# TopJohn/corda

Hardware: AMD Instinct MI355X
Metric: signature verifications/sec (whole node, 1/2/4/8 GPU) + % integer-ALU peak (higher is better)
Workload: dtype u32

## Files before the change

### corda_amd/csrc/ed25519.hip

```cpp
#ifndef FE_QUAD
#define FE_QUAD 0
#endif
#ifndef FE_USE_ASM2
#define FE_USE_ASM2 1
#endif
#include <hip/hip_runtime.h>

#include <functional>
#include <stdint.h>
#include <stdlib.h>

#include "ed25519_half.hpp"
#include "ed25519_ops.hpp"
#include "ed25519_route.hpp"
#include "ed25519_ws.hpp"
#include "sha2_device.hpp"
#include "status.hpp"

namespace cordahip {

__global__ void __launch_bounds__(64) ed25519_btable_kernel(uint32_t* __restrict__ tab) {
  const int g = blockIdx.x * blockDim.x + threadIdx.x;
  if (g >= 2 * kBTableEntries) return;
  const int k = g % kBTableEntries;
  ge_p3 B, P;
  ge_base(B);
  if (g >= kBTableEntries)
    for (int t = 0; t < kBDigits * kBBits; t++) ge_dbl<true>(B, B);
  ge_cached bc;
  ge_to_cached(bc, B);
  ge_identity(P);
  for (int bit = kBBits - 1; bit >= 0; bit--) {
    ge_dbl<true>(P, P);
    if ((k >> bit) & 1) ge_add<true>(P, P, bc);
  }
  store_niels_entry(tab + g * kBEntryWords, P);
  if (g == 0) {
    ge_cached id;
    fe_set(id.YpX, 1);
    fe_set(id.YmX, 1);
    fe_set(id.Z, 1);
    fe_set(id.T2d, 0);
    store_cached(tab + kBIdentityWord, id);
  }
}


CDEV double mp8_top(const uint32_t a[8], int s) {
  const int w = s >> 5, b = s & 31;
  const uint64_t lo = ((uint64_t)word_sel(a, w + 1) << 32) | word_sel(a, w);
  const uint64_t hi = word_sel(a, w + 2);
  return (double)((lo >> b) | (b ? hi << (64 - b) : 0ull));
}
CDEV void mp8_lincomb(uint32_t o[8], const uint32_t x[8], int a, const uint32_t y[8], int b) {
  const uint32_t ua = (uint32_t)(a < 0 ? -a : a), ub = (uint32_t)(b < 0 ? -b : b);
  uint64_t pc = 0, qc = 0;
  uint32_t br = 0;
#pragma unroll
  for (int i = 0; i < 8; i++) {
    const uint64_t p = (uint64_t)ua * x[i] + pc;
    pc = p >> 32;
    const uint64_t q = (uint64_t)ub * y[i] + qc;
    qc = q >> 32;
    const uint64_t d = (uint64_t)(uint32_t)p - (uint32_t)q - br;
    o[i] = (uint32_t)d;
    br = (uint32_t)(d >> 63);
  }
  if (b > 0 || (b == 0 && a < 0)) mp8_neg(o);
}

CDEV void half_scalars(uint32_t c0abs[8], bool& c0neg, uint32_t c1[8], const uint32_t h[8]) {
  const uint32_t kM[8] = {0xe7ae9f68u, 0xc09318d2u, 0x17bce6b2u, 0xa6f7cef5u, 0u, 0u, 0u, 0x80000000u};
  const uint32_t kS[8] = {0x754abea0u, 0x597d89b3u, 0xf9de6484u, 0xb504f333u, 0u, 0u, 0u, 0u};
  uint32_t rp[8], rc[8], tp[8], tc[8];
#pragma unroll
  for (int i = 0; i < 8; i++) {
    rp[i] = kM[i];
    rc[i] = h[i];
    tp[i] = 0;
    tc[i] = i == 0;
  }
  for (;;) {
    const int s = max(mp8_bitlen(rp) - 52, 0);
    double uh = mp8_top(rp, s), vh = mp8_top(rc, s);
    const double th = mp8_top(kS, s) + 1.0;
    double A = 1.0, B = 0.0, C = 0.0, D = 1.0;
    int n = 0;
    for (;;) {
      const double d1 = vh + C, d2 = vh + D;
      if (!(d1 > 0.0 && d2 > 0.0)) break;
      const double n1 = uh + A;
      double q = floor(n1 / d1);
      const double r1 = fma(-q, d1, n1);
      q = r1 < 0.0 ? q - 1.0 : (r1 >= d1 ? q + 1.0 : q);
      const double r2 = fma(-q, d2, uh + B);
      if (!(r2 >= 0.0 && r2 < d2)) break;
      const double nC = fma(-q, C, A), nD = fma(-q, D, B), nv = fma(-q, vh, uh);
      const double mc = fmax(fabs(nC), fabs(nD));
      if (nv - mc < th || mc >= 0x1p30) break;
      A = C;
      B = D;
      C = nC;
      D = nD;
      uh = vh;
      vh = nv;
      n++;
    }
    if (n == 0) break;
    const int a = (int)A, b = (int)B, c = (int)C, d = (int)D;
    uint32_t x[8], y[8];
    mp8_lincomb(x, rp, a, rc, b);
// ... 172 lines not shown
  ge_to_cached(c, E);
  store_cached(joint_slot(rec, joint_index(2, 2 * s)), c);
}


#ifndef ED_PREP_WAVES
#define ED_PREP_WAVES 2
#endif
CDEV uint8_t prep_decode_phase(const uint8_t* __restrict__ keys, const uint8_t* __restrict__ sigs, uint64_t i,
                               uint32_t msg_len, const uint8_t* __restrict__ pre_status, uint32_t empty_is_error,
                               uint32_t* __restrict__ rec, uint32_t* col, uint32_t abyte[8], uint32_t Rw[8]) {
  uint8_t st = kStatusPending;
  load8(Rw, reinterpret_cast<const uint32_t*>(sigs + i * 64));
  {
    uint32_t wa[8];
    load8(wa, reinterpret_cast<const uint32_t*>(keys + i * 32));
    ge_p3 A, R;
    bool okA, okR;
    ge_frombytes_i2p_pair(A, okA, wa, R, okR, Rw);
    if (!okA) st = kStatusBadKey;
    else if (pre_status && pre_status[i] != kStatusOk) st = pre_status[i];
    else if (msg_len == 0 && empty_is_error) st = kStatusEmpty;
    fe_tobytes(abyte, A.Y);
    abyte[7] |= fe_isnegative(A.X) << 31;
    if (st == kStatusPending && !(okR && ge_strict_ok(R, Rw))) st = kStatusBadSig;
    if (st != kStatusPending) {
      ge_identity(A);
      ge_identity(R);
    }
    fe_neg(A.X, A.X);
    fe_neg(A.T, A.T);
    fe_neg(R.X, R.X);
    fe_neg(R.T, R.T);
    park_point(rec, col, 0, A);
    park_point(rec, col, 1, R);
  }
  return st;
}

CDEV void prep_table_phase(uint32_t* __restrict__ rec, uint32_t* col) {
#pragma unroll 1
  for (int pass = 0; pass < 2; pass++) {
    joint_single_pass(rec, col, pass);
    PHASE_BARRIER();
  }
#pragma unroll 1
  for (int s = -1; s <= 1; s += 2) {
    joint_sign_pass(rec, col, s);
    PHASE_BARRIER();
  }
}

CDEV uint8_t prep_keys_phase(const uint8_t* __restrict__ keys, const uint8_t* __restrict__ sigs, uint64_t i,
                             uint32_t msg_len, const uint8_t* __restrict__ pre_status, uint32_t empty_is_error,
                             uint32_t* __restrict__ rec, uint32_t* col, uint32_t abyte[8], uint32_t Rw[8]) {
  const uint8_t st = prep_decode_phase(keys, sigs, i, msg_len, pre_status, empty_is_error, rec, col, abyte, Rw);
  PHASE_BARRIER();
  prep_table_phase(rec, col);
  return st;
}

CDEV void prep_msg_phase(const uint8_t* __restrict__ sigs, const uint8_t* __restrict__ msgs, uint32_t msg_len,
                         uint64_t i, uint8_t st, const uint32_t abyte[8], const uint32_t Rw[8],
                         uint32_t* __restrict__ rec) {
  uint32_t ka[8], kr[8], e[8];
  bool c0neg = false;
  if (st == kStatusPending) {
    uint32_t S[8], hd[16], h[8], se[8], zero[8];
    load8(S, reinterpret_cast<const uint32_t*>(sigs + i * 64 + 32));
    sha512_segments(hd, Rw, abyte, true, msgs + i * (uint64_t)msg_len, msg_len);
    sc_reduce512(h, hd);
    sc_effective_S(se, S, slide_drops_carry(S));
    half_scalars(ka, c0neg, kr, h);
#pragma unroll
    for (int q = 0; q < 8; q++) zero[q] = 0;
    sc_muladd(e, kr, se, zero);
  } else {
#pragma unroll
    for (int q = 0; q < 8; q++) ka[q] = kr[q] = e[q] = 0;
  }
#if ED_SEL_STREAM
  uint32_t sel[32];
  sel_recode(sel, ka, kr, e, c0neg);
  sel[kSelWords] = 0;
  uint4* o4 = reinterpret_cast<uint4*>(rec + kWhSel);
#pragma unroll
  for (int q = 0; q < 8; q++) o4[q] = make_uint4(sel[4 * q], sel[4 * q + 1], sel[4 * q + 2], sel[4 * q + 3]);
#else
  store8(rec + kWhKa, ka);
  store8(rec + kWhKr, kr);
  store8(rec + kWhE, e);
  reinterpret_cast<uint4*>(rec + kWhFlags)[0] = make_uint4(c0neg ? 1u : 0u, 0u, 0u, 0u);
#endif
}

#if ED_PREP_LDS
#define PREP_PARK_COLUMN(col)                  \
  __shared__ uint32_t pq_lds[kPqWords][256]; \
  uint32_t* col = &pq_lds[0][threadIdx.x]
#else
#define PREP_PARK_COLUMN(col) uint32_t* col = nullptr
#endif

__global__ void __launch_bounds__(256) __attribute__((amdgpu_waves_per_eu(ED_PREP_WAVES))) ed25519_prep_half_kernel(
    const uint8_t* __restrict__ keys, const uint8_t* __restrict__ sigs, const uint8_t* __restrict__ msgs,
    uint32_t msg_len, uint64_t base, uint64_t m, const uint8_t* __restrict__ pre_status,
    uint8_t* __restrict__ status, uint32_t* __restrict__ ws, uint32_t empty_is_error) {
  const uint64_t li = (uint64_t)blockIdx.x * blockDim.x + threadIdx.x;
  if (li >= m) return;
  const uint64_t i = base + li;
  uint32_t* rec = ws + li * kWhLaneWords;
  uint32_t abyte[8], Rw[8];
  PREP_PARK_COLUMN(col);
  const uint8_t st = prep_keys_phase(keys, sigs, i, msg_len, pre_status, empty_is_error, rec, col, abyte, Rw);
  prep_msg_phase(sigs, msgs, msg_len, i, st, abyte, Rw, rec);
  status[i] = st;
}

__global__ void __launch_bounds__(256) __attribute__((amdgpu_waves_per_eu(ED_PREP_WAVES)))
ed25519_prep_half_idx_kernel(const uint8_t* __restrict__ keys, const uint8_t* __restrict__ sigs,
                             const uint8_t* __restrict__ msgs, uint32_t msg_len, uint64_t base, uint64_t m,
                             const uint8_t* __restrict__ pre_status, uint8_t* __restrict__ status,
                             uint32_t* __restrict__ ws, uint32_t empty_is_error, const uint32_t* __restrict__ scratch,
                             uint64_t lanes) {
  const uint64_t li = (uint64_t)blockIdx.x * blockDim.x + threadIdx.x;
  if (li >= route_chunk_lanes(scratch[kRouteCntGeneric], base, m)) return;
  const uint64_t i = scratch[route_off_generic(lanes) + base + li];
  uint32_t* rec = ws + li * kWhLaneWords;
  uint32_t abyte[8], Rw[8];
  PREP_PARK_COLUMN(col);
  const uint8_t st = prep_keys_phase(keys, sigs, i, msg_len, pre_status, empty_is_error, rec, col, abyte, Rw);
  prep_msg_phase(sigs, msgs, msg_len, i, st, abyte, Rw, rec);
  status[i] = st;
}

__global__ void __launch_bounds__(256) __attribute__((amdgpu_waves_per_eu(ED_PREP_WAVES))) ed25519_prep_keys_kernel(
    const uint8_t* __restrict__ keys, const uint8_t* __restrict__ sigs, uint32_t msg_len, uint64_t base, uint64_t m,
    const uint8_t* __restrict__ pre_status, uint8_t* __restrict__ status, uint32_t* __restrict__ ws,
    uint32_t empty_is_error) {
  const uint64_t li = (uint64_t)blockIdx.x * blockDim.x + threadIdx.x;
  if (li >= m) return;
  const uint64_t i = base + li;
  uint32_t* rec = ws + li * kWhLaneWords;
  uint32_t abyte[8], Rw[8];
  PREP_PARK_COLUMN(col);
  status[i] = prep_keys_phase(keys, sigs, i, msg_len, pre_status, empty_is_error, rec, col, abyte, Rw);
  store8(rec + kWhKa, abyte);
}

__global__ void __launch_bounds__(256) __attribute__((amdgpu_waves_per_eu(ED_PREP_WAVES))) ed25519_prep_msg_kernel(const uint8_t* __restrict__ sigs,
                                                               const uint8_t* __restrict__ msgs, uint32_t msg_len,
                                                               uint64_t base, uint64_t m,
                                                               const uint8_t* __restrict__ status,
                                                               uint32_t* __restrict__ ws) {
  const uint64_t li = (uint64_t)blockIdx.x * blockDim.x + threadIdx.x;
  if (li >= m) return;
  const uint64_t i = base + li;
  uint32_t* rec = ws + li * kWhLaneWords;
  uint32_t abyte[8], Rw[8];
  load8(abyte, rec + kWhKa);
  load8(Rw, reinterpret_cast<const uint32_t*>(sigs + i * 64));
  prep_msg_phase(sigs, msgs, msg_len, i, status[i], abyte, Rw, rec);
}

CDEV void fixed_base_mult(ge_p3& P, const uint32_t k[8], const uint32_t* __restrict__ btab) {
  ge_identity(P);
  for (int j = 31; j >= 0; j--) {
// ... 143 lines not shown
```

### corda_amd/csrc/ed25519_ladder.hip

```cpp
#ifndef FE_USE_ASM2
#define FE_USE_ASM2 1
#endif
#include <hip/hip_runtime.h>
#include <stdint.h>

#include "ed25519_route.hpp"
#include "ed25519_ws.hpp"
#include "status.hpp"

namespace cordahip {

__device__ __attribute__((aligned(64))) const uint32_t kIdentityCached[kWhEntryWords] = {1, 0, 0, 0, 0, 0, 0, 0, 0, 0,
                                                            1, 0, 0, 0, 0, 0, 0, 0, 0, 0,
                                                            1, 0, 0, 0, 0, 0, 0, 0, 0, 0,
                                                            0, 0, 0, 0, 0, 0, 0, 0, 0, 0};

#ifndef ED_LADDER_WAVES
#define ED_LADDER_WAVES 2
#endif
static_assert(512 / ED_LADDER_WAVES >= 168, "fe25519_asm.hpp's v160..v167 accumulators need >= 168 VGPRs per lane");

#ifndef ED_LADDER_ORDER
#define ED_LADDER_ORDER 1
#endif
#if ED_LADDER_ORDER && !ED_SEL_STREAM
#error "ED_LADDER_ORDER ranks the lanes by the selector stream's window count"
#endif
static constexpr int kOrderLo = 60, kOrderHi = 74, kOrderKeys = kOrderHi - kOrderLo + 2;
static_assert(kOrderKeys <= 64, "one lane of a wave per key");

template <bool kIdx>
CDEV void ladder_half_lane(uint64_t base, uint64_t m, const uint32_t* __restrict__ btab,
                           const uint32_t* __restrict__ ws, uint8_t* __restrict__ status,
                           unsigned long long* __restrict__ verdict, const uint32_t* __restrict__ list) {
  const uint64_t blk = (uint64_t)blockIdx.x * blockDim.x;
#if ED_LADDER_ORDER
  __shared__ uint32_t sk[kSelWords][256];
  __shared__ uint8_t order_src[256];
  __shared__ uint32_t order_cnt[4][kOrderKeys];
  __shared__ uint32_t order_done;
  uint64_t li;
  {
    const uint64_t l0 = blk + threadIdx.x;
    const uint32_t* r0 = ws + (l0 < m ? l0 : m - 1) * kWhLaneWords;
    const uint4* r4 = reinterpret_cast<const uint4*>(r0 + kWhSel);
    uint4 v[(kSelWords + 3) / 4];
#pragma unroll
    for (int q = 0; q < (kSelWords + 3) / 4; q++) v[q] = r4[q];
    static_assert(kSelMeta == 30 && (kSelWords + 3) / 4 == 8, "the count is in the last quad's third word");
    const int cnt = (int)(v[7].z >> 16);
    const int key = l0 < m ? min(max(cnt, kOrderLo), kOrderHi) - kOrderLo : kOrderKeys - 1;
    const int lane = threadIdx.x & 63, wave = threadIdx.x >> 6;
    uint32_t before = 0, mine = 0;
#pragma unroll
    for (int k = 0; k < kOrderKeys; k++) {
      const unsigned long long mk = __ballot(key == k);
      if (key == k) before = (uint32_t)__popcll(mk & ((1ull << lane) - 1));
      if (lane == k) mine = (uint32_t)__popcll(mk);
    }
    if (lane < kOrderKeys) order_cnt[wave][lane] = mine;
    if (threadIdx.x == 0) order_done = 0;
    __syncthreads();
    uint32_t rank = before;
#pragma unroll
    for (int k = 0; k < kOrderKeys; k++)
#pragma unroll
      for (int w = 0; w < 4; w++) {
        const uint32_t c = order_cnt[w][k];
        rank += (k < key || (k == key && w < wave)) ? c : 0u;
      }
    order_src[rank] = (uint8_t)threadIdx.x;
#pragma unroll
    for (int q = 0; q < (kSelWords + 3) / 4; q++) {
      const uint32_t w[4] = {v[q].x, v[q].y, v[q].z, v[q].w};
#pragma unroll
      for (int t = 0; t < 4; t++)
        if (4 * q + t < kSelWords) sk[4 * q + t][rank] = w[t];
    }
    __syncthreads();
    li = blk + order_src[threadIdx.x];
  }
#else
  const uint64_t li = blk + threadIdx.x;
#endif
  const bool active = li < m;
  const uint64_t lc = active ? li : m - 1;
  const uint32_t* rec = ws + lc * kWhLaneWords;
#if ED_IDENT_GLOBAL
  const uint32_t* ident = btab + kBIdentityWord;
#else
  const uint32_t* ident = kIdentityCached;
#endif
  const uint32_t* btab2 = btab + kBTableEntries * kBEntryWords;
  ge_p3 P;
  ge_identity(P);
#if ED_SEL_STREAM
#if !ED_LADDER_ORDER
  __shared__ uint32_t sk[kSelWords][256];
  {
    const uint4* r4 = reinterpret_cast<const uint4*>(rec + kWhSel);
#pragma unroll
    for (int q = 0; q < (kSelWords + 3) / 4; q++) {
      const uint4 v = r4[q];
      const uint32_t w[4] = {v.x, v.y, v.z, v.w};
#pragma unroll
      for (int t = 0; t < 4; t++)
        if (4 * q + t < kSelWords) sk[4 * q + t][threadIdx.x] = w[t];
    }
  }
#endif
  const uint32_t* col = &sk[0][threadIdx.x];
#if ED_LADDER_ORDER
  const int own = active ? (int)(col[kSelMeta * 256] >> 16) : 0;
#else
  const int own = (int)(col[kSelMeta * 256] >> 16);
#endif
  const int W = min(max(wave_max(own), (kBDigits - 1) * (kBBits / 2) + 1), kSelWindows);
  uint32_t selw = col[((W - 1) / kSelPerWord) * 256];
  for (int j = W - 1; j >= 0; j--) {
    const int jn = max(j - 1, 0);
    const uint32_t selw_next = col[(jn / kSelPerWord) * 256];
    const uint32_t sel = selw >> (kSelBits * (j % kSelPerWord));
    const uint32_t idx = sel & 15u;
    const bool neg = sel & kSelNeg;
    ge_cached c;
    load_cached(c, idx == kSelIdentity ? ident : rec + kWhTab + idx * kWhEntryWords);
    const bool bwin = j % (kBBits / 2) == 0 && j < kBDigits * (kBBits / 2);
    uint32_t m0 = 0, m1 = 0, sg = 0;
    const int t = j / (kBBits / 2);
    if (bwin) {
      m0 = col[(kSelMag + (t >> 1)) * 256];
      m1 = col[(kSelMag + ((t + kBDigits) >> 1)) * 256];
      sg = col[kSelMeta * 256];
    }
    if (j != W - 1) {
      ge_dbl<false>(P, P);
      ge_dbl<true>(P, P);
    }
    cached_cneg(c, neg);
    if (bwin) {
      const int sh = 16 * (t & 1);
      ge_niels nb0, nb1;
      uint32_t pad0[2], pad1[2];
      load_niels(nb0, btab, (int)((m0 >> sh) & 0xffffu), pad0);
      ge_add<true>(P, P, c);
      load_niels(nb1, btab2, (int)((m1 >> sh) & 0xffffu), pad1);
      niels_pad_use(pad0);
      niels_cneg(nb0, (sg >> t) & 1u);
      ge_madd<true>(P, P, nb0);
      niels_pad_use(pad1);
      niels_cneg(nb1, (sg >> (t + kBDigits)) & 1u);
      ge_madd<false>(P, P, nb1);
    } else {
      ge_add<false>(P, P, c);
    }
    selw = selw_next;
  }
#else
  __shared__ uint32_t sk[24][256];
  const uint32_t* ska = &sk[0][threadIdx.x];
  const uint32_t* skr = &sk[8][threadIdx.x];
  const uint32_t* ske = &sk[16][threadIdx.x];
  int bits;
  {
    uint32_t ka[8], kr[8], e[8];
    load8(ka, rec + kWhKa);
    load8(kr, rec + kWhKr);
    load8(e, rec + kWhE);
#pragma unroll
    for (int q = 0; q < 8; q++) {
      sk[q][threadIdx.x] = ka[q];
      sk[8 + q][threadIdx.x] = kr[q];
      sk[16 + q][threadIdx.x] = e[q];
    }
    bits = max(mp8_bitlen(ka), mp8_bitlen(kr));
  }
  const bool c0neg = rec[kWhFlags] & 1u;
  const int W = max(wave_max((bits + 2) / 2), (kBDigits - 1) * (kBBits / 2) + 1);
  for (int j = W - 1; j >= 0; j--) {
    const joint_sel sel = joint_select(joint_booth2(ska, 256, 8, j), joint_booth2(skr, 256, 8, j), c0neg);
    ge_cached c;
    load_cached(c, table_entry(rec, sel.idx, ident));
    if (j != W - 1) {
      ge_dbl<false>(P, P);
      ge_dbl<true>(P, P);
    }
    cached_cneg(c, sel.neg);
    const bool bwin = j % (kBBits / 2) == 0 && j < kBDigits * (kBBits / 2);
    if (bwin) {
      const int d0 = booth_digit_col<kBBits>(ske, j / (kBBits / 2));
      const int d1 = booth_digit_col<kBBits>(ske, j / (kBBits / 2) + kBDigits);
      ge_niels nb0, nb1;
      load_niels(nb0, btab, d0 < 0 ? -d0 : d0);
      ge_add<true>(P, P, c);
      load_niels(nb1, btab2, d1 < 0 ? -d1 : d1);
      niels_cneg(nb0, d0 < 0);
      ge_madd<true>(P, P, nb0);
      niels_cneg(nb1, d1 < 0);
      ge_madd<false>(P, P, nb1);
    } else {
      ge_add<false>(P, P, c);
    }
  }
#endif
  fe d;
  fe_sub(d, P.Y, P.Z);
  const bool zero = fe_iszero(P.X) && fe_iszero(d);
  const uint64_t i = kIdx ? (active ? list[base + li] : 0) : base + li;
  uint8_t st = kStatusBadSig;
  if (active) {
    st = status[i];
    if (st == kStatusPending) {
      st = zero ? kStatusOk : kStatusBadSig;
      status[i] = st;
    }
  }
  if (!kIdx) {
#if ED_LADDER_ORDER
    __shared__ uint8_t order_ok[256];
    order_ok[li - blk] = active && st == kStatusOk;
    __builtin_amdgcn_fence(__ATOMIC_RELEASE, "workgroup");
    uint32_t arrived = 0;
    if ((threadIdx.x & 63) == 0)
      arrived = __hip_atomic_fetch_add(&order_done, 1u, __ATOMIC_RELAXED, __HIP_MEMORY_SCOPE_WORKGROUP);
    arrived = (uint32_t)__shfl((int)arrived, 0);
    if (arrived == blockDim.x / 64 - 1) {
      __builtin_amdgcn_fence(__ATOMIC_ACQUIRE, "workgroup");
      const int lane = threadIdx.x & 63;
#pragma unroll
      for (int q = 0; q < 4; q++) {
        const unsigned long long ok = __ballot(order_ok[64 * q + lane] != 0);
        if (lane == q && blk + 64 * q < m && verdict) verdict[(base + blk + 64 * q) >> 6] = ok;
      }
    }
#else
    const unsigned long long ok = __ballot(active && st == kStatusOk);
    if ((threadIdx.x & 63) == 0 && active && verdict) verdict[i >> 6] = ok;
#endif
  }
}

__global__ void __launch_bounds__(256) __attribute__((amdgpu_waves_per_eu(ED_LADDER_WAVES))) ed25519_ladder_half_kernel(
    uint64_t base, uint64_t m, const uint32_t* __restrict__ btab, const uint32_t* __restrict__ ws,
    uint8_t* __restrict__ status, unsigned long long* __restrict__ verdict) {
  ladder_half_lane<false>(base, m, btab, ws, status, verdict, nullptr);
}

__global__ void __launch_bounds__(256) __attribute__((amdgpu_waves_per_eu(ED_LADDER_WAVES)))
ed25519_ladder_half_idx_kernel(uint64_t base, uint64_t m, const uint32_t* __restrict__ btab,
                               const uint32_t* __restrict__ ws, uint8_t* __restrict__ status,
                               const uint32_t* __restrict__ scratch, uint64_t lanes) {
  const uint64_t mm = route_chunk_lanes(scratch[kRouteCntGeneric], base, m);
  if ((uint64_t)blockIdx.x * blockDim.x >= mm) return;
  ladder_half_lane<true>(base, mm, btab, ws, status, nullptr, scratch + route_off_generic(lanes));
}

hipError_t launch_ed25519_ladder(uint64_t base, uint64_t m, const uint32_t* btab, const uint32_t* ws, uint8_t* status,
                                 unsigned long long* verdict, hipStream_t s) {
  const uint32_t blocks = (uint32_t)((m + 255) / 256);
  hipLaunchKernelGGL(ed25519_ladder_half_kernel, dim3(blocks), dim3(256), 0, s, base, m, btab, ws, status, verdict);
  return hipGetLastError();
}

hipError_t launch_ed25519_ladder_idx(uint64_t base, uint64_t m, const uint32_t* btab, const uint32_t* ws,
                                     uint8_t* status, const uint32_t* scratch, uint64_t lanes, hipStream_t s) {
  const uint32_t blocks = (uint32_t)((m + 255) / 256);
  hipLaunchKernelGGL(ed25519_ladder_half_idx_kernel, dim3(blocks), dim3(256), 0, s, base, m, btab, ws, status, scratch,
                     lanes);
  return hipGetLastError();
}

}
```

### corda_amd/csrc/ed25519_sel.hpp

```cpp
#pragma once
#include <stdint.h>

#include "ed25519_joint.hpp"

namespace cordahip {

static constexpr int kSelPerWord = 6, kSelBits = 5;
static constexpr int kSelWindows = 132;
static constexpr uint32_t kSelIdentity = 15;
static constexpr uint32_t kSelNeg = 16;
static constexpr int kSelBDigits = 16;
static constexpr int kSelMag = kSelWindows / kSelPerWord;
static constexpr int kSelMeta = kSelMag + kSelBDigits / 2;
static constexpr int kSelWords = kSelMeta + 1;
static constexpr int kSelAlways = 80;
static_assert(kSelWindows % kSelPerWord == 0 && kSelWindows >= 129 && kSelWords <= 32,
              "the stream lives in the record's 32 scalar words");

static constexpr uint32_t kBooth2Lut = 2u | 3u << 3 | 3u << 6 | 4u << 9 | 0u << 12 | 1u << 15 | 1u << 18 | 2u << 21;

JOINT_HD uint32_t sel_byte(uint32_t va, uint32_t vr) {
  const int ta = (int)((kBooth2Lut >> (3 * va)) & 7u), tr = (int)((kBooth2Lut >> (3 * vr)) & 7u);
  const int s = 5 * ta + tr - 12;
  const int m = s < 0 ? -s : s;
  return ((uint32_t)(m - 1) & 15u) | (s < 0 ? kSelNeg : 0u);
}
static_assert(((uint32_t)kJointIdentity & 15u) == kSelIdentity && kJointEntries <= (int)kSelIdentity &&
                  (kSelNeg | 15u) < (1u << kSelBits),
              "selector encoding");

JOINT_HD void sel_word(uint32_t out[kSelWords], int w, uint32_t a, uint32_t r, uint32_t pa, uint32_t pr) {
#pragma unroll
  for (int b = 0; b < 16; b++) {
    const int j = 16 * w + b;
    if (j >= kSelWindows) break;
    const uint32_t va = b ? (a >> (2 * b - 1)) & 7u : ((a << 1) | pa) & 7u;
    const uint32_t vr = b ? (r >> (2 * b - 1)) & 7u : ((r << 1) | pr) & 7u;
    const int sh = kSelBits * (j % kSelPerWord);
    out[j / kSelPerWord] ^= (sel_byte(va, vr) ^ (j >= kSelAlways ? kSelIdentity : 0u)) << sh;
  }
}

JOINT_HD void sel_recode(uint32_t out[kSelWords], const uint32_t c0abs[8], const uint32_t c1[8], const uint32_t e[8],
                         bool c0neg) {
  const uint32_t flip = c0neg ? ~0u : 0u;
#pragma unroll
  for (int k = 0; k < kSelMag; k++) {
    uint32_t v = 0;
#pragma unroll
    for (int t = 0; t < kSelPerWord; t++)
      if (kSelPerWord * k + t >= kSelAlways) v |= kSelIdentity << (kSelBits * t);
    out[k] = v;
  }
#pragma unroll
  for (int w = 0; w < kSelAlways / 16; w++)
    sel_word(out, w, c0abs[w] ^ flip, c1[w], w ? (c0abs[w - 1] ^ flip) >> 31 : flip >> 31, w ? c1[w - 1] >> 31 : 0u);
  const uint32_t high = (c0abs[4] | c1[4]) >> 31 | c0abs[5] | c1[5] | c0abs[6] | c1[6] | c0abs[7] | c1[7];
  if (high) {
#pragma unroll
    for (int w = kSelAlways / 16; w <= 8; w++)
      sel_word(out, w, (w < 8 ? c0abs[w] : 0u) ^ flip, w < 8 ? c1[w] : 0u, (c0abs[w - 1] ^ flip) >> 31, c1[w - 1] >> 31);
  }
  uint32_t signs = 0;
#pragma unroll
  for (int w = 0; w < kSelBDigits / 2; w++) {
    const uint32_t v0 = ((e[w] << 1) | (w ? e[w - 1] >> 31 : 0u)) & 0x1ffffu, v1 = e[w] >> 15;
    const int d0 = (int)((v0 + 1) >> 1) - (int)((v0 >> 16) << 16), d1 = (int)((v1 + 1) >> 1) - (int)((v1 >> 16) << 16);
    signs |= (d0 < 0 ? 1u : 0u) << (2 * w) | (d1 < 0 ? 1u : 0u) << (2 * w + 1);
    out[kSelMag + w] = (uint32_t)(d0 < 0 ? -d0 : d0) | (uint32_t)(d1 < 0 ? -d1 : d1) << 16;
  }
  int bits = 0;
#pragma unroll
  for (int i = 0; i < 8; i++) {
    const uint32_t m = c0abs[i] | c1[i];
    bits = m ? 32 * i + 32 - __builtin_clz(m) : bits;
  }
  out[kSelMeta] = signs | (uint32_t)((bits + 2) / 2) << 16;
}

JOINT_HD uint32_t sel_window(const uint32_t s[kSelWords], int j) {
  return (s[j / kSelPerWord] >> (kSelBits * (j % kSelPerWord))) & ((1u << kSelBits) - 1);
}
JOINT_HD int sel_count(const uint32_t s[kSelWords]) { return (int)((s[kSelMeta] >> 16) & 0xffu); }
JOINT_HD int sel_bdigit(const uint32_t s[kSelWords], int t) {
  const int mag = (int)((s[kSelMag + (t >> 1)] >> (16 * (t & 1))) & 0xffffu);
  return (s[kSelMeta] >> t) & 1u ? -mag : mag;
}

}
```

### corda_amd/csrc/ed25519_ws.hpp

```cpp
#pragma once
#include "ed25519_joint.hpp"
#include "ed25519_sel.hpp"
#include "fe25519.hpp"
#include "ge25519.hpp"
#include "sc25519.hpp"

namespace cordahip {

static constexpr int kBBits = 16;
static constexpr int kBDigits = 8;
static constexpr int kBTableEntries = (1 << (kBBits - 1)) + 1;
static constexpr int kBEntryWords = 32;
static constexpr int kBIdentityWord = 2 * kBTableEntries * kBEntryWords;
static_assert(kSelBDigits == 2 * kBDigits, "ed25519_sel.hpp recodes both halves of e");
static constexpr uint8_t kStatusPending = 0xff;

#ifndef ED_SEL_STREAM
#define ED_SEL_STREAM 1
#endif
#ifndef ED_IDENT_GLOBAL
#define ED_IDENT_GLOBAL 1
#endif
static constexpr int kWhEntryWords = 48;
static constexpr int kWhTab = 0;
static constexpr int kWhKa = kJointEntries * kWhEntryWords;
static constexpr int kWhKr = kWhKa + 8;
static constexpr int kWhE = kWhKa + 16;
static constexpr int kWhFlags = kWhKa + 24;
static constexpr int kWhLaneWords = kWhKa + 32;
static_assert(kWhLaneWords % 16 == 0, "records must start on 64-B sectors");

static constexpr int kWhSel = kWhKa;

extern __device__ const uint32_t kIdentityCached[kWhEntryWords];

CDEV const uint32_t* table_entry(const uint32_t* rec, int idx, const uint32_t* ident) {
  return idx == kJointIdentity ? ident : rec + kWhTab + idx * kWhEntryWords;
}

CDEV void load_niels(ge_niels& n, const uint32_t* __restrict__ tab, int idx, uint32_t pad[2]) {
  const uint4* e = reinterpret_cast<const uint4*>(tab + idx * kBEntryWords);
  uint32_t w[32];
#pragma unroll
  for (int q = 0; q < 8; q++) {
    const uint4 v = e[q];
    w[4 * q] = v.x;
    w[4 * q + 1] = v.y;
    w[4 * q + 2] = v.z;
    w[4 * q + 3] = v.w;
  }
#pragma unroll
  for (int i = 0; i < 10; i++) {
    n.ypx.v[i] = w[i];
    n.ymx.v[i] = w[10 + i];
    n.xy2d.v[i] = w[20 + i];
  }
  pad[0] = w[30];
  pad[1] = w[31];
}
CDEV void load_niels(ge_niels& n, const uint32_t* __restrict__ tab, int idx) {
  uint32_t pad[2];
  load_niels(n, tab, idx, pad);
}
#ifndef ED_NIELS_PAD_LIVE
#define ED_NIELS_PAD_LIVE 1
#endif
CDEV void niels_pad_use(const uint32_t pad[2]) {
#if ED_NIELS_PAD_LIVE
  asm volatile("" ::"v"(pad[0]), "v"(pad[1]));
#endif
}

CDEV void niels_cneg(ge_niels& n, bool neg) {
  fe nt;
  fe_neg_loose(nt, n.xy2d);
#pragma unroll
  for (int i = 0; i < 10; i++) {
    const uint32_t a = n.ypx.v[i], b = n.ymx.v[i];
    n.ypx.v[i] = neg ? b : a;
    n.ymx.v[i] = neg ? a : b;
    n.xy2d.v[i] = neg ? nt.v[i] : n.xy2d.v[i];
  }
}
CDEV void cached_cneg(ge_cached& c, bool neg) {
  fe nt;
  fe_neg_loose(nt, c.T2d);
#pragma unroll
  for (int i = 0; i < 10; i++) {
    const uint32_t a = c.YpX.v[i], b = c.YmX.v[i];
    c.YpX.v[i] = neg ? b : a;
    c.YmX.v[i] = neg ? a : b;
    c.T2d.v[i] = neg ? nt.v[i] : c.T2d.v[i];
  }
}

CDEV void store_cached(uint32_t* __restrict__ o, const ge_cached& c) {
  uint4* o4 = reinterpret_cast<uint4*>(o);
// ... 80 lines not shown
```

### corda_amd/csrc/ge25519.hpp

```cpp
#pragma once
#include "fe25519.hpp"
#if FE_USE_ASM2
#include "fe25519_asm.hpp"
#endif

namespace cordahip {

#ifndef FE_USE_ASM2
#define FE_USE_ASM2 0
#endif
CDEV void fe_mul_pair(fe& r0, const fe& f0, const fe& g0, fe& r1, const fe& f1, const fe& g1) {
#if FE_USE_ASM2
  fe_mul2(r0, f0, g0, r1, f1, g1);
#else
  fe o0, o1;
  fe_mul(o0, f0, g0);
  fe_mul(o1, f1, g1);
  r0 = o0;
  r1 = o1;
#endif
}
CDEV void fe_sq_pair(fe& r0, const fe& f0, fe& r1, const fe& f1) {
#if FE_USE_ASM2
  fe_sq2(r0, f0, r1, f1);
// ... 30 lines not shown
  fe_mul_pair(o2, f2, g2, o3, f3, g3);
  fe_mul_pair(r0, f0, g0, r1, f1, g1);
  r2 = o2;
  r3 = o3;
#endif
}
template <bool WANT_T, class P>
CDEV void ge_out_stage(P& r, const fe& f, const fe& e, const fe& g, const fe& h) {
#if FE_USE_ASM2 && FE_QUAD
  if (WANT_T) fe_mul4x(r.X, r.Y, r.Z, r.T, f, h, e, g);
  else fe_mul3x(r.X, r.Y, r.Z, f, h, e, g);
#else
  if (WANT_T) fe_mul_quad(r.X, f, e, r.Y, g, h, r.Z, f, g, r.T, e, h);
  else fe_mul_triple(r.X, f, e, r.Y, g, h, r.Z, f, g);
#endif
}

struct ge_p3 {
  fe X, Y, Z, T;
};
struct ge_cached {
  fe YpX, YmX, Z, T2d;
};
struct ge_niels {
  fe ypx, ymx, xy2d;
};

CDEV void ge_identity(ge_p3& r) {
  fe_set(r.X, 0);
  fe_set(r.Y, 1);
  fe_set(r.Z, 1);
  fe_set(r.T, 0);
}

CDEV void ge_to_cached(ge_cached& c, const ge_p3& p) {
  fe d2;
  fe_const_d2(d2);
  fe_add(c.YpX, p.Y, p.X);
  fe_sub(c.YmX, p.Y, p.X);
  c.Z = p.Z;
  fe_mul(c.T2d, p.T, d2);
}

template <bool WANT_T>
CDEV void ge_dbl(ge_p3& r, const ge_p3& p) {
  fe a, b, c, e, f, g, h, t;
  fe_add(t, p.X, p.Y);
  fe_sq_pair(a, p.X, b, p.Y);
  fe_sq_pair(c, p.Z, t, t);
  fe_add(h, a, b);
  fe_sub(e, h, t);
  fe_sub_loose(g, a, b);
  fe_add(f, c, c);
  fe_add(f, f, g);
  ge_out_stage<WANT_T>(r, f, e, g, h);
}

template <bool WANT_T>
CDEV void ge_add(ge_p3& r, const ge_p3& p, const ge_cached& q) {
  fe a, b, c, d, e, f, g, h, t, u;
  fe_sub_loose(t, p.Y, p.X);
  fe_add(u, p.Y, p.X);
  fe_mul_quad(a, t, q.YmX, b, u, q.YpX, c, p.T, q.T2d, d, p.Z, q.Z);
  fe_add(d, d, d);
  fe_sub_loose(e, b, a);
  fe_sub_loose(f, d, c);
  fe_add(g, d, c);
  fe_add(h, b, a);
  ge_out_stage<WANT_T>(r, f, e, g, h);
}

template <bool WANT_T>
CDEV void ge_madd(ge_p3& r, const ge_p3& p, const ge_niels& q) {
  fe a, b, c, d, e, f, g, h, t, u;
  fe_sub_loose(t, p.Y, p.X);
  fe_add(u, p.Y, p.X);
  fe_mul_triple(a, t, q.ymx, b, u, q.ypx, c, p.T, q.xy2d);
  fe_add(d, p.Z, p.Z);
  fe_sub_loose(e, b, a);
  fe_sub_loose(f, d, c);
  fe_add(g, d, c);
  fe_add(h, b, a);
  ge_out_stage<WANT_T>(r, f, e, g, h);
}

CDEV void ge_tobytes(uint32_t w[8], const ge_p3& p) {
  fe zi, x, y;
  fe_invert(zi, p.Z);
  fe_mul(x, p.X, zi);
  fe_mul(y, p.Y, zi);
  fe_tobytes(w, y);
  w[7] ^= fe_isnegative(x) << 31;
}

CDEV bool ge_frombytes_i2p(ge_p3& r, const uint32_t w[8]) {
  fe y, yy, u, v, v3, x, vxx, chk, dd, one;
  fe_set(one, 1);
  fe_const_d(dd);
  fe_frombytes(y, w);
  fe_sq(yy, y);
  fe_sub(u, yy, one);
  fe_mul(v, yy, dd);
  fe_add(v, v, one);
  fe_sq(v3, v);
  fe_mul(v3, v3, v);
  fe_sq(x, v3);
  fe_mul(x, x, v);
  fe_mul(x, x, u);
  fe_pow22523(x, x);
  fe_mul(x, x, v3);
  fe_mul(x, x, u);
  fe_sq(vxx, x);
  fe_mul(vxx, vxx, v);
  fe_sub(chk, vxx, u);
  bool ok = true;
  if (!fe_iszero(chk)) {
    fe_add(chk, vxx, u);
    if (!fe_iszero(chk)) {
      ok = false;
    } else {
      fe i;
      fe_const_sqrtm1(i);
      fe_mul(x, x, i);
    }
  }
  if (fe_isnegative(x) != (w[7] >> 31)) fe_neg(x, x);
  r.X = x;
  r.Y = y;
  fe_set(r.Z, 1);
  fe_mul(r.T, x, y);
  return ok;
}

CDEV void fe_sqn_pair(fe& r0, const fe& a0, fe& r1, const fe& a1, int n) {
  fe_sq_pair(r0, a0, r1, a1);
#pragma unroll 1
  for (int i = 1; i < n; i++) fe_sq_pair(r0, r0, r1, r1);
}
CDEV void fe_pow22523_pair(fe& r0, const fe& z0, fe& r1, const fe& z1) {
  fe z2_0, z2_1, z9_0, z9_1, z11_0, z11_1, t0, t1, a0, a1, b0, b1;
  fe_sq_pair(z2_0, z0, z2_1, z1);
  fe_sqn_pair(t0, z2_0, t1, z2_1, 2);
  fe_mul_pair(z9_0, t0, z0, z9_1, t1, z1);
  fe_mul_pair(z11_0, z9_0, z2_0, z11_1, z9_1, z2_1);
  fe_sq_pair(t0, z11_0, t1, z11_1);
  fe_mul_pair(a0, t0, z9_0, a1, t1, z9_1);
  fe_sqn_pair(t0, a0, t1, a1, 5);
  fe_mul_pair(a0, t0, a0, a1, t1, a1);
  fe_sqn_pair(t0, a0, t1, a1, 10);
  fe_mul_pair(b0, t0, a0, b1, t1, a1);
  fe_sqn_pair(t0, b0, t1, b1, 20);
  fe_mul_pair(t0, t0, b0, t1, t1, b1);
  fe_sqn_pair(t0, t0, t1, t1, 10);
  fe_mul_pair(a0, t0, a0, a1, t1, a1);
  fe_sqn_pair(t0, a0, t1, a1, 50);
  fe_mul_pair(b0, t0, a0, b1, t1, a1);
  fe_sqn_pair(t0, b0, t1, b1, 100);
  fe_mul_pair(t0, t0, b0, t1, t1, b1);
  fe_sqn_pair(t0, t0, t1, t1, 50);
  fe_mul_pair(t0, t0, a0, t1, t1, a1);
  fe_sqn_pair(t0, t0, t1, t1, 2);
  fe_mul_pair(r0, t0, z0, r1, t1, z1);
}

CDEV void ge_frombytes_i2p_pair(ge_p3& r0, bool& ok0, const uint32_t w0[8], ge_p3& r1, bool& ok1,
                                const uint32_t w1[8]) {
// ... 50 lines not shown
```

Measured before the change: 120.9 million.

## Widen fixed-base comb to 20-bit digits and trim top/bottom ladder steps

Makes the fixed-base B table digit width configurable (default 20 bits instead of 16). This cuts the number of fixed-base niels additions; in windows that lack a high digit the ladder does one madd instead of two. The first window now initialises P directly from the cached entry rather than adding it to the identity. The final madd is replaced by an identity test that skips computing the full point. The cost is larger B tables (2^19 entries per half), worse cache locality for random table gathers, and more complex bit-packed magnitude extraction.

```diff
diff --git a/corda_amd/csrc/ed25519.hip b/corda_amd/csrc/ed25519.hip
--- a/corda_amd/csrc/ed25519.hip
+++ b/corda_amd/csrc/ed25519.hip
@@ -26,7 +26,7 @@
   ge_p3 B, P;
   ge_base(B);
   if (g >= kBTableEntries)
-    for (int t = 0; t < kBDigits * kBBits; t++) ge_dbl<true>(B, B);
+    for (int t = 0; t < kBDigitsLo * kBBits; t++) ge_dbl<true>(B, B);
   ge_cached bc;
   ge_to_cached(bc, B);
   ge_identity(P);
@@ -365,7 +365,8 @@
 #if ED_SEL_STREAM
   uint32_t sel[32];
   sel_recode(sel, ka, kr, e, c0neg);
-  sel[kSelWords] = 0;
+#pragma unroll
+  for (int q = kSelWords; q < 32; q++) sel[q] = 0;
   uint4* o4 = reinterpret_cast<uint4*>(rec + kWhSel);
 #pragma unroll
   for (int q = 0; q < 8; q++) o4[q] = make_uint4(sel[4 * q], sel[4 * q + 1], sel[4 * q + 2], sel[4 * q + 3]);
diff --git a/corda_amd/csrc/ed25519_ladder.hip b/corda_amd/csrc/ed25519_ladder.hip
--- a/corda_amd/csrc/ed25519_ladder.hip
+++ b/corda_amd/csrc/ed25519_ladder.hip
@@ -25,6 +25,12 @@
 #endif
 #if ED_LADDER_ORDER && !ED_SEL_STREAM
 #error "ED_LADDER_ORDER ranks the lanes by the selector stream's window count"
+#endif
+#ifndef ED_LADDER_TOP_LOAD
+#define ED_LADDER_TOP_LOAD 1
+#endif
+#ifndef ED_LADDER_LAST_EH
+#define ED_LADDER_LAST_EH 1
 #endif
 static constexpr int kOrderLo = 60, kOrderHi = 74, kOrderKeys = kOrderHi - kOrderLo + 2;
 static_assert(kOrderKeys <= 64, "one lane of a wave per key");
@@ -47,8 +53,10 @@
     uint4 v[(kSelWords + 3) / 4];
 #pragma unroll
     for (int q = 0; q < (kSelWords + 3) / 4; q++) v[q] = r4[q];
-    static_assert(kSelMeta == 30 && (kSelWords + 3) / 4 == 8, "the count is in the last quad's third word");
-    const int cnt = (int)(v[7].z >> 16);
+    static_assert(kSelMeta / 4 == 7 && (kSelWords + 3) / 4 == 8, "the count is in the last quad");
+    const uint32_t meta = kSelMeta % 4 == 2 ? v[7].z : v[7].w;
+    static_assert(kSelMeta % 4 >= 2, "its third or fourth word");
+    const int cnt = (int)(meta >> 16);
     const int key = l0 < m ? min(max(cnt, kOrderLo), kOrderHi) - kOrderLo : kOrderKeys - 1;
     const int lane = threadIdx.x & 63, wave = threadIdx.x >> 6;
     uint32_t before = 0, mine = 0;
@@ -115,7 +123,8 @@
 #else
   const int own = (int)(col[kSelMeta * 256] >> 16);
 #endif
-  const int W = min(max(wave_max(own), (kBDigits - 1) * (kBBits / 2) + 1), kSelWindows);
+  const int W = min(max(wave_max(own), kBMinWindows), kSelWindows);
+  bool zero = false;
   uint32_t selw = col[((W - 1) / kSelPerWord) * 256];
   for (int j = W - 1; j >= 0; j--) {
     const int jn = max(j - 1, 0);
@@ -125,38 +134,56 @@
     const bool neg = sel & kSelNeg;
     ge_cached c;
     load_cached(c, idx == kSelIdentity ? ident : rec + kWhTab + idx * kWhEntryWords);
-    const bool bwin = j % (kBBits / 2) == 0 && j < kBDigits * (kBBits / 2);
+    const bool bwin = j % kBWin == 0 && j < kBDigitsLo * kBWin;
+    const int t = j / kBWin;
+    const bool hi = t < kBDigitsHi;
     uint32_t m0 = 0, m1 = 0, sg = 0;
-    const int t = j / (kBBits / 2);
     if (bwin) {
-      m0 = col[(kSelMag + (t >> 1)) * 256];
-      m1 = col[(kSelMag + ((t + kBDigits) >> 1)) * 256];
+      m0 = sel_bmag(col, 256, t);
+      if (hi) m1 = sel_bmag(col, 256, t + kBDigitsLo);
       sg = col[kSelMeta * 256];
     }
-    if (j != W - 1) {
+    const bool top = j == W - 1;
+    if (!top) {
       ge_dbl<false>(P, P);
       ge_dbl<true>(P, P);
     }
     cached_cneg(c, neg);
     if (bwin) {
-      const int sh = 16 * (t & 1);
-      ge_niels nb0, nb1;
-      uint32_t pad0[2], pad1[2];
-      load_niels(nb0, btab, (int)((m0 >> sh) & 0xffffu), pad0);
+      ge_niels nb;
+      uint32_t pad[2];
+      bool nbneg = sel_bneg(sg, hi ? t + kBDigitsLo : t);
+      load_niels(nb, hi ? btab2 : btab, (int)(hi ? m1 : m0), pad);
       ge_add<true>(P, P, c);
-      load_niels(nb1, btab2, (int)((m1 >> sh) & 0xffffu), pad1);
-      niels_pad_use(pad0);
-      niels_cneg(nb0, (sg >> t) & 1u);
-      ge_madd<true>(P, P, nb0);
-      niels_pad_use(pad1);
-      niels_cneg(nb1, (sg >> (t + kBDigits)) & 1u);
-      ge_madd<false>(P, P, nb1);
+      if (hi) {
+        ge_niels nb0;
+        uint32_t pad0[2];
+        load_niels(nb0, btab, (int)m0, pad0);
+        niels_pad_use(pad);
+        niels_cneg(nb, nbneg);
+        ge_madd<true>(P, P, nb);
+        nb = nb0;
+        pad[0] = pad0[0];
+        pad[1] = pad0[1];
+        nbneg = sel_bneg(sg, t);
+      }
+      niels_pad_use(pad);
+      niels_cneg(nb, nbneg);
+#if ED_LADDER_LAST_EH
+      if (j == 0) zero = ge_madd_is_identity(P, nb);
+      else ge_madd<false>(P, P, nb);
+#else
+      ge_madd<false>(P, P, nb);
+#endif
+    } else if (ED_LADDER_TOP_LOAD && top) {
+      ge_from_cached(P, c);
     } else {
       ge_add<false>(P, P, c);
     }
     selw = selw_next;
   }
 #else
+  static_assert(kBBits == 16 && kBDigitsLo == kBDigitsHi, "without the selector stream the ladder is 16-bit only");
   __shared__ uint32_t sk[24][256];
   const uint32_t* ska = &sk[0][threadIdx.x];
   const uint32_t* skr = &sk[8][threadIdx.x];
@@ -176,7 +203,7 @@
     bits = max(mp8_bitlen(ka), mp8_bitlen(kr));
   }
   const bool c0neg = rec[kWhFlags] & 1u;
-  const int W = max(wave_max((bits + 2) / 2), (kBDigits - 1) * (kBBits / 2) + 1);
+  const int W = max(wave_max((bits + 2) / 2), kBMinWindows);
   for (int j = W - 1; j >= 0; j--) {
     const joint_sel sel = joint_select(joint_booth2(ska, 256, 8, j), joint_booth2(skr, 256, 8, j), c0neg);
     ge_cached c;
@@ -186,10 +213,10 @@
       ge_dbl<true>(P, P);
     }
     cached_cneg(c, sel.neg);
-    const bool bwin = j % (kBBits / 2) == 0 && j < kBDigits * (kBBits / 2);
+    const bool bwin = j % (kBBits / 2) == 0 && j < kBDigitsLo * (kBBits / 2);
     if (bwin) {
       const int d0 = booth_digit_col<kBBits>(ske, j / (kBBits / 2));
-      const int d1 = booth_digit_col<kBBits>(ske, j / (kBBits / 2) + kBDigits);
+      const int d1 = booth_digit_col<kBBits>(ske, j / (kBBits / 2) + kBDigitsLo);
       ge_niels nb0, nb1;
       load_niels(nb0, btab, d0 < 0 ? -d0 : d0);
       ge_add<true>(P, P, c);
@@ -202,10 +229,17 @@
       ge_add<false>(P, P, c);
     }
   }
-#endif
   fe d;
   fe_sub(d, P.Y, P.Z);
   const bool zero = fe_iszero(P.X) && fe_iszero(d);
+#endif
+#if ED_SEL_STREAM && !ED_LADDER_LAST_EH
+  {
+    fe d;
+    fe_sub(d, P.Y, P.Z);
+    zero = fe_iszero(P.X) && fe_iszero(d);
+  }
+#endif
   const uint64_t i = kIdx ? (active ? list[base + li] : 0) : base + li;
   uint8_t st = kStatusBadSig;
   if (active) {
diff --git a/corda_amd/csrc/ed25519_sel.hpp b/corda_amd/csrc/ed25519_sel.hpp
--- a/corda_amd/csrc/ed25519_sel.hpp
+++ b/corda_amd/csrc/ed25519_sel.hpp
@@ -9,10 +9,24 @@
 static constexpr int kSelWindows = 132;
 static constexpr uint32_t kSelIdentity = 15;
 static constexpr uint32_t kSelNeg = 16;
-static constexpr int kSelBDigits = 16;
+#ifndef ED_B_BITS
+#define ED_B_BITS 20
+#endif
+static constexpr int kBBits = ED_B_BITS;
+static_assert(kBBits == 16 || kBBits == 18 || kBBits == 20, "ED_B_BITS: 16, 18 or 20");
+static constexpr int kBWin = kBBits / 2;
+static constexpr int kBDigitsLo = 63 / kBWin + 1;
+static constexpr int kBDigitsHi = (254 + kBBits - 1) / kBBits - kBDigitsLo;
+static constexpr int kBDigits = kBDigitsLo + kBDigitsHi;
+static constexpr int kBMinWindows = (kBDigitsLo - 1) * kBWin + 1;
+static_assert(kBDigits * kBBits >= 254, "e < 2^253 and the Booth carry");
+static_assert(kBMinWindows <= 64, "the digits force no window a normal lane does not have");
+static_assert(kBDigitsHi >= 1 && kBDigitsHi <= kBDigitsLo, "a window's high digit has a low digit beside it");
 static constexpr int kSelMag = kSelWindows / kSelPerWord;
-static constexpr int kSelMeta = kSelMag + kSelBDigits / 2;
+static constexpr int kSelMagWords = (kBDigits * kBBits + 31) / 32;
+static constexpr int kSelMeta = kSelMag + kSelMagWords;
 static constexpr int kSelWords = kSelMeta + 1;
+static_assert(kBDigits <= 16, "the meta word's sign bits");
 static constexpr int kSelAlways = 80;
 static_assert(kSelWindows % kSelPerWord == 0 && kSelWindows >= 129 && kSelWords <= 32,
               "the stream lives in the record's 32 scalar words");
@@ -63,11 +77,19 @@
   }
   uint32_t signs = 0;
 #pragma unroll
-  for (int w = 0; w < kSelBDigits / 2; w++) {
-    const uint32_t v0 = ((e[w] << 1) | (w ? e[w - 1] >> 31 : 0u)) & 0x1ffffu, v1 = e[w] >> 15;
-    const int d0 = (int)((v0 + 1) >> 1) - (int)((v0 >> 16) << 16), d1 = (int)((v1 + 1) >> 1) - (int)((v1 >> 16) << 16);
-    signs |= (d0 < 0 ? 1u : 0u) << (2 * w) | (d1 < 0 ? 1u : 0u) << (2 * w + 1);
-    out[kSelMag + w] = (uint32_t)(d0 < 0 ? -d0 : d0) | (uint32_t)(d1 < 0 ? -d1 : d1) << 16;
+  for (int w = 0; w < kSelMagWords; w++) out[kSelMag + w] = 0;
+#pragma unroll
+  for (int t = 0; t < kBDigits; t++) {
+    const int lo = kBBits * t - 1, w = lo < 0 ? 0 : lo >> 5, sh = lo < 0 ? 0 : lo & 31;
+    uint32_t v = lo < 0 ? e[0] << 1 : e[w] >> sh;
+    if (sh && w + 1 < 8) v |= e[w + 1] << (32 - sh);
+    v &= (2u << kBBits) - 1;
+    const int d = (int)((v + 1) >> 1) - (int)((v >> kBBits) << kBBits);
+    const uint32_t mag = (uint32_t)(d < 0 ? -d : d);
+    signs |= (d < 0 ? 1u : 0u) << t;
+    const int ow = (kBBits * t) >> 5, osh = (kBBits * t) & 31;
+    out[kSelMag + ow] |= mag << osh;
+    if (osh + kBBits > 32) out[kSelMag + ow + 1] |= mag >> (32 - osh);
   }
   int bits = 0;
 #pragma unroll
@@ -82,9 +104,15 @@
   return (s[j / kSelPerWord] >> (kSelBits * (j % kSelPerWord))) & ((1u << kSelBits) - 1);
 }
 JOINT_HD int sel_count(const uint32_t s[kSelWords]) { return (int)((s[kSelMeta] >> 16) & 0xffu); }
+JOINT_HD uint32_t sel_bmag(const uint32_t* s, int stride, int t) {
+  const int w = kSelMag + ((kBBits * t) >> 5), sh = (kBBits * t) & 31;
+  const uint64_t two = (uint64_t)s[(w + 1) * stride] << 32 | s[w * stride];
+  return (uint32_t)(two >> sh) & ((1u << kBBits) - 1);
+}
+JOINT_HD bool sel_bneg(uint32_t meta, int t) { return (meta >> t) & 1u; }
 JOINT_HD int sel_bdigit(const uint32_t s[kSelWords], int t) {
-  const int mag = (int)((s[kSelMag + (t >> 1)] >> (16 * (t & 1))) & 0xffffu);
-  return (s[kSelMeta] >> t) & 1u ? -mag : mag;
+  const int mag = (int)sel_bmag(s, 1, t);
+  return sel_bneg(s[kSelMeta], t) ? -mag : mag;
 }
 
 }
diff --git a/corda_amd/csrc/ed25519_ws.hpp b/corda_amd/csrc/ed25519_ws.hpp
--- a/corda_amd/csrc/ed25519_ws.hpp
+++ b/corda_amd/csrc/ed25519_ws.hpp
@@ -7,12 +7,10 @@
 
 namespace cordahip {
 
-static constexpr int kBBits = 16;
-static constexpr int kBDigits = 8;
 static constexpr int kBTableEntries = (1 << (kBBits - 1)) + 1;
 static constexpr int kBEntryWords = 32;
 static constexpr int kBIdentityWord = 2 * kBTableEntries * kBEntryWords;
-static_assert(kSelBDigits == 2 * kBDigits, "ed25519_sel.hpp recodes both halves of e");
+static_assert((long long)2 * kBTableEntries * kBEntryWords + 64 < (1ll << 31), "table word offsets are ints");
 static constexpr uint8_t kStatusPending = 0xff;
 
 #ifndef ED_SEL_STREAM
diff --git a/corda_amd/csrc/ge25519.hpp b/corda_amd/csrc/ge25519.hpp
--- a/corda_amd/csrc/ge25519.hpp
+++ b/corda_amd/csrc/ge25519.hpp
@@ -136,6 +136,27 @@
   fe_add(g, d, c);
   fe_add(h, b, a);
   ge_out_stage<WANT_T>(r, f, e, g, h);
+}
+
+CDEV bool ge_madd_is_identity(const ge_p3& p, const ge_niels& q) {
+  fe a, b, c, d, e, s, t, u;
+  fe_sub_loose(t, p.Y, p.X);
+  fe_add(u, p.Y, p.X);
+  fe_mul_triple(a, t, q.ymx, b, u, q.ypx, c, p.T, q.xy2d);
+  fe_sub(e, b, a);
+  fe_add(s, b, a);
+  fe_add(s, s, c);
+  fe_add(d, p.Z, p.Z);
+  fe_sub(s, s, d);
+  return fe_iszero(e) && fe_iszero(s);
+}
+
+CDEV void ge_from_cached(ge_p3& r, const ge_cached& q) {
+  fe_sub(r.X, q.YpX, q.YmX);
+  fe_add(r.Y, q.YpX, q.YmX);
+  fe_carry(r.Y);
+  fe_add(r.Z, q.Z, q.Z);
+  fe_carry(r.Z);
 }
 
 CDEV void ge_tobytes(uint32_t w[8], const ge_p3& p) {
```

Result: faster. 122.3 million, median of 6 (+1.1%).
